# IIT-PAVIS/Acoustic-Image-Generation

Measured on AMD Instinct MI355X. Metric: train-step images/sec, higher is better.
Workload: dtype f32

## Files before the change

### acoustic-image-generation_amd/csrc/igemm.hip

```cpp
#include "wgrad_split3_kernel.hpp"
#include "igemm_split3d_kernel.hpp"
#include "igemm_split3dp_kernel.hpp"
#include "igemm_split3r_kernel.hpp"
#include "igemm_split3h_kernel.hpp"
#include "skinny_kernel.hpp"
#include <cstdlib>
#include <algorithm>
#include <type_traits>

namespace acimg {

__global__ __launch_bounds__(256) void igemm_splitk_reduce_kernel(const float* slab, int splits,
                                                                  int M, int Ngemm, int slab_ld,
                                                                  const EpiParams e) {
    const long idx = (long)blockIdx.x * 256 + threadIdx.x;
    const long total = (long)M * Ngemm;
    if (idx >= total) return;
    const int m = (int)(idx / Ngemm);
    const int n = (int)(idx - (long)m * Ngemm);
    float v = 0.f;
    for (int z = 0; z < splits; ++z) v += slab[((long)z * M + m) * slab_ld + n];
    if (n >= e.Nstore) return;
    int cn, pixoff, r, q, oh, ow;
    epi_col(e, n, cn, pixoff, r, q);
    const long rp = epi_row_pix(e, m, oh, ow);
    if (epi_lands(e, oh, ow, r, q)) epi_store(e, rp + pixoff, cn, v);
}

__global__ __launch_bounds__(256) void subpixel_weights_kernel(const float* w, int R, int S, int Ko, int Kin, int ldw, int U,
                                                               int V, float* wc, int total) {
    const int idx = blockIdx.x * 256 + threadIdx.x;
    if (idx >= total) return;
    const int ncol = 4 * Ko;
    const int row = idx / ncol, col = idx - row * ncol;
    const int kin = row % Kin, tap = row / Kin;
    const int up = tap / V, vp = tap - up * V;
    const int cls = col / Ko, ko = col - cls * Ko;
    const int a = cls >> 1, b = cls & 1;
    const int r = a + 2 * (U - 1 - up), q = b + 2 * (V - 1 - vp);
    wc[idx] = (r < R && q < S) ? w[((long)(r * S + q) * Ko + ko) * ldw + kin] : 0.f;
}

template <int BMO, int BN, int WGM = 2>
__global__ __launch_bounds__(256) void wgrad_f32_kernel(const WgradParams p) {
    constexpr int BKR = 16;
    constexpr int LDA_S = BMO + 4;
    constexpr int LDB_S = BN + 4;
    constexpr int WGN = 4 / WGM;
    constexpr int WTM = BMO / WGM, WTN = BN / WGN;
    static_assert(WTM % 16 == 0 && WTN % 16 == 0, "wave tile");
    constexpr int TM = WTM / 16, TN = WTN / 16;
    constexpr int AQ = BMO / 4;
    constexpr int ARPP = 256 / AQ;
    constexpr int NA = (BKR + ARPP - 1) / ARPP;
    constexpr int BQ = BN / 4;
    constexpr int BRPP = 256 / BQ;
    constexpr int NB = (BKR + BRPP - 1) / BRPP;

    __shared__ __attribute__((aligned(16))) float As[BKR * LDA_S];
    __shared__ __attribute__((aligned(16))) float Bs[BKR * LDB_S];

    const int tid = threadIdx.x;
    const int lane = tid & 63, wid = tid >> 6;
    const int wm = wid / WGN, wn = wid % WGN;
    const int li = lane & 15, g = lane >> 4;
    const int kk0 = blockIdx.x * BMO, n0 = blockIdx.y * BN;

    const int m_begin = blockIdx.z * p.rows_per_split;
    const int m_end = min(p.M, m_begin + p.rows_per_split);

    const int aq = tid % AQ;
    const int arow0 = tid / AQ;
    const int kk = kk0 + aq * 4;
    const bool kk_ok = kk < p.KK;
    const bool kk_ones = p.db_out != nullptr && kk == p.KK;
    int r = 0, s = 0, c = 0;
    if (kk_ok) {
        const int tap = kk / p.C;
        c = kk - tap * p.C;
        r = tap / p.S;
        s = tap - r * p.S;
    }
    const int bq = tid % BQ;
    const int brow0 = tid / BQ;
    const int nb = n0 + bq * 4;
    const bool nb_ok = nb < p.Nld;
    const int ohw = p.OH * p.OW;

    int x_img[NA], x_oh[NA], x_ow[NA];
#pragma unroll
    for (int j = 0; j < NA; ++j) {
        const int m = m_begin + arow0 + j * ARPP;
        x_img[j] = m / ohw;
        const int rem = m - x_img[j] * ohw;
        x_oh[j] = rem / p.OW;
        x_ow[j] = rem - x_oh[j] * p.OW;
    }

    float4 ra[NA], rb[NB];
    auto load_tiles = [&](int mb) {
#pragma unroll
        for (int j = 0; j < NA; ++j) {
            const int row = arow0 + j * ARPP;
            const int m = mb + row;
            float4 v = make_float4(0.f, 0.f, 0.f, 0.f);
            if (row < BKR && kk_ones && m < m_end) v.x = 1.f;
            if (row < BKR && kk_ok && m < m_end) {
                const int ih = x_oh[j] * p.stride - p.pad_t + r;
                const int iw = x_ow[j] * p.stride - p.pad_l + s;
                if ((unsigned)ih < (unsigned)p.H && (unsigned)iw < (unsigned)p.W)
                    v = *reinterpret_cast<const float4*>(
                        p.X + ((long)(x_img[j] * p.H + ih) * p.W + iw) * p.ldx + c);
            }
            ra[j] = v;
            x_ow[j] += BKR;
            while (x_ow[j] >= p.OW) {
                x_ow[j] -= p.OW;
                if (++x_oh[j] == p.OH) {
                    x_oh[j] = 0;
                    ++x_img[j];
                }
            }
        }
#pragma unroll
        for (int j = 0; j < NB; ++j) {
            const int row = brow0 + j * BRPP;
            const int m = mb + row;
            float4 v = make_float4(0.f, 0.f, 0.f, 0.f);
            if (row < BKR && nb_ok && m < m_end)
                v = *reinterpret_cast<const float4*>(p.G + (long)m * p.ldg + nb);
            rb[j] = v;
        }
    };
    auto store_tiles = [&]() {
#pragma unroll
        for (int j = 0; j < NA; ++j) {
            const int row = arow0 + j * ARPP;
            if (row < BKR) *reinterpret_cast<float4*>(&As[row * LDA_S + aq * 4]) = ra[j];
        }
#pragma unroll
        for (int j = 0; j < NB; ++j) {
            const int row = brow0 + j * BRPP;
            if (row < BKR) *reinterpret_cast<float4*>(&Bs[row * LDB_S + bq * 4]) = rb[j];
        }
    };

    f32x4 acc[TM][TN];
#pragma unroll
    for (int i = 0; i < TM; ++i)
#pragma unroll
        for (int j = 0; j < TN; ++j) acc[i][j] = f32x4{0.f, 0.f, 0.f, 0.f};

    if (m_begin < m_end) {
// ... 508 lines not shown
    if (s <= 1) return 0;
    const int ld = (Ngemm + 3) & ~3;
    const size_t rows = (size_t)s * M * ld * sizeof(float);
    const size_t tiled = (size_t)s * cdiv(M, c.bm) * cdiv(Ngemm, c.bn) * c.bm * c.bn * sizeof(float);
    return rows > tiled ? rows : tiled;
}

template <int BM, int BN, int WGM, int WGN, int NTHR>
static void launch_cfg(const IgemmParams& p, bool nt, bool cal, dim3 grid, hipStream_t st) {
    constexpr int BK = 32;
    constexpr int a_elems = BM * (BK + 4);
    constexpr int bnt = BN * (BK + 4), bnn = BK * (BN + 4);
    const int stage = a_elems + (nt ? bnt : bnn);
    const int stat_elems = WGM * 2 * BN;
    const int elems = 2 * stage > stat_elems ? 2 * stage : stat_elems;
    const size_t shm = (size_t)elems * sizeof(float);
    if (nt) {
        if (cal) hipLaunchKernelGGL((igemm_f32_kernel<BM, BN, WGM, WGN, NTHR, true, true>), grid, dim3(NTHR), shm, st, p);
        else hipLaunchKernelGGL((igemm_f32_kernel<BM, BN, WGM, WGN, NTHR, true, false>), grid, dim3(NTHR), shm, st, p);
    } else {
        if (cal) hipLaunchKernelGGL((igemm_f32_kernel<BM, BN, WGM, WGN, NTHR, false, true>), grid, dim3(NTHR), shm, st, p);
        else hipLaunchKernelGGL((igemm_f32_kernel<BM, BN, WGM, WGN, NTHR, false, false>), grid, dim3(NTHR), shm, st, p);
    }
}

static void epi_vec_flag(EpiParams& e) {
    e.vec = aligned16(e.Y) && (e.ldy & 3) == 0 && (!e.bias || aligned16(e.bias)) &&
            (!e.res || (aligned16(e.res) && (e.ldres & 3) == 0)) &&
            (!e.mask || (aligned16(e.mask) && (e.ldmask & 3) == 0)) && (!e.scatter || (e.Ko & 3) == 0);
}

static IgemmParams fwd_view(const AcimgConvDesc* d) {
    IgemmParams p{};
    p.H = d->H; p.W = d->W; p.C = d->C; p.lda = d->ldx;
    p.OH = d->OH; p.OW = d->OW; p.R = d->R; p.S = d->S; p.stride = d->stride;
    p.pad_t = d->pad_t; p.pad_l = d->pad_l;
    p.M = d->N * d->OH * d->OW;
    p.Nld = d->ldw; p.Ngemm = d->K;
    p.e.ldy = d->ldy; p.e.M = p.M; p.e.Nstore = d->K; p.e.act = d->act; p.e.stats_ld = d->ldw;
    return p;
}
static IgemmParams flipped_view(int N, int GH, int GW, int ca, int ldgy, int H, int W, int R, int S, int pad_t, int pad_l,
                                int cols) {
    IgemmParams p{};
    p.H = GH; p.W = GW; p.C = ca; p.lda = ldgy;
    p.OH = H; p.OW = W; p.R = R; p.S = S; p.stride = 1;
    p.pad_t = R - 1 - pad_t; p.pad_l = S - 1 - pad_l;
    p.M = N * H * W;
    p.Ngemm = cols;
    p.e.M = p.M; p.e.Nstore = cols; p.e.act = ACIMG_ACT_NONE;
    return p;
}
static IgemmParams flipped_view(const AcimgConvDesc* d, int ca, int ldgy) {
    return flipped_view(d->N, d->OH, d->OW, ca, ldgy, d->H, d->W, d->R, d->S, d->pad_t, d->pad_l, d->C);
}
static void split_ksteps(IgemmParams& p) {
    p.ntaps = p.R * p.S;
    p.kiters = p.ntaps * (p.C / 32);
    p.splits = 1;
}

static int launch_igemm(IgemmParams p, bool nt, void* ws, size_t ws_bytes, void* tickets, hipStream_t st) {
    if (p.M <= 0 || p.Ngemm <= 0) return fail(ACIMG_EINVAL, "igemm: empty problem");
    if ((p.C & 3) || (p.lda & 3) || (p.ldb & 3))
        return fail(ACIMG_EINVAL, "igemm: C=%d lda=%d ldb=%d must be multiples of 4", p.C, p.lda, p.ldb);
    if (!aligned16(p.A) || !aligned16(p.B)) return fail(ACIMG_EINVAL, "igemm: operands must be 16-byte aligned");
    const int nseg = p.rowrun ? p.R : p.R * p.S;
    p.L = p.rowrun ? p.S * p.C : p.C;
    p.cps = cdiv(p.L, 32);
    p.kiters = nseg * p.cps;
    p.ntaps = p.R * p.S;
    const bool cal = (p.C % 32) == 0;
    const long nimg = p.M / ((long)p.OH * p.OW);
    const long a_bytes = ((nimg * p.H * p.W - 1) * p.lda + p.C) * 4;
    const long b_bytes = nt ? (((long)(p.ntaps - 1) * p.tap_stride + (long)(p.Ngemm - 1) * p.ldb + p.C) * 4)
                            : ((long)p.R * p.S * p.C * p.ldb * 4);
    if (a_bytes >= (1L << 31) || b_bytes >= (1L << 31) || a_bytes <= 0 || b_bytes <= 0)
        return fail(ACIMG_EINVAL, "igemm: operand extent %ld / %ld bytes outside (0, 2 GiB)", a_bytes, b_bytes);
    p.a_bytes = (unsigned)a_bytes;
    p.b_bytes = (unsigned)b_bytes;
    EpiParams& e = p.e;
    epi_vec_flag(e);
    TileCfg c = pick_cfg(p.M, p.Ngemm);
    p.splits = pick_splits(p.M, p.Ngemm, c, p.kiters);
    float* stats_after = nullptr;
    if (e.stats && p.splits > 1) {
        if (e.scatter || e.res || e.mask || e.act != ACIMG_ACT_NONE)
            return fail(ACIMG_EINVAL, "igemm: statistics with split-K need a raw (conv + bias) output");
        stats_after = e.stats;
        e.stats = nullptr;
    }
    p.slab = nullptr;
    p.slab_ld = (p.Ngemm + 3) & ~3;
    p.ts_counters = nullptr;
    dim3 grid(cdiv(p.M, c.bm), cdiv(p.Ngemm, c.bn), p.splits);
    if (p.splits > 1) {
        size_t need = (size_t)p.splits * p.M * p.slab_ld * sizeof(float);
        const size_t tiles = (size_t)grid.x * grid.y;
        if (tickets && (reinterpret_cast<uintptr_t>(tickets) & 15))
            return fail(ACIMG_EINVAL, "igemm: ticket words must be 16-byte aligned");
        const bool handoff = tickets != nullptr && tiles <= ACIMG_TICKET_WORDS && g_cfg.splitk_handoff;
        if (handoff) need = (size_t)p.splits * tiles * c.bm * c.bn * sizeof(float);
        if (ws == nullptr || ws_bytes < need)
            return fail(ACIMG_EWORKSPACE, "igemm: workspace %zu < %zu", ws_bytes, need);
        p.slab = static_cast<float*>(ws);
        if (handoff) p.ts_counters = static_cast<int*>(tickets);
    }
    if (c.bm == 128 && c.bn == 128) launch_cfg<128, 128, 2, 4, 512>(p, nt, cal, grid, st);
    else if (c.bm == 128 && c.bn == 64) launch_cfg<128, 64, 2, 2, 256>(p, nt, cal, grid, st);
    else if (c.bm == 64 && c.bn == 64) launch_cfg<64, 64, 2, 2, 256>(p, nt, cal, grid, st);
    else launch_cfg<256, 16, 4, 1, 256>(p, nt, cal, grid, st);
    int rc = check_launch("igemm");
    if (rc) return rc;
    if (p.splits > 1) {
        if (p.ts_counters == nullptr) {
            const long total = (long)p.M * p.Ngemm;
            hipLaunchKernelGGL(igemm_splitk_reduce_kernel, dim3(cdiv(total, 256)), dim3(256), 0, st,
                               p.slab, p.splits, p.M, p.Ngemm, p.slab_ld, p.e);
            rc = check_launch("igemm_splitk_reduce");
        }
        if (!rc && stats_after) {
            hipLaunchKernelGGL(partial_stats_kernel, dim3(cdiv(p.M, 256)), dim3(256), 0, st, e.Y, e.ldy, p.M,
                               e.Nstore, stats_after, e.stats_ld, 256);
            rc = check_launch("partial_stats");
        }
    }
    return rc;
}

static int pick_wgrad_splits(int M, int KK, int Ngemm, int bmo, int bn) {
    const long tiles = (long)cdiv(KK, bmo) * cdiv(Ngemm, bn);
    long s = (512 + tiles - 1) / tiles;
    const int minpix = g_cfg.wgrad_minpix;
    const long maxs = (M + minpix - 1) / minpix;
    long cap = 128;
    if ((long)KK * Ngemm <= 8192) {
        s = (2048 + tiles - 1) / tiles;
        cap = 2048;
    }
    if (s > maxs) s = maxs;
    if (s > cap) s = cap;
    if (s < 1) s = 1;
    return (int)s;
}
static void wgrad_tile(int Ngemm, int& bmo, int& bn) {
    bmo = 128;
    bn = Ngemm <= 16 ? 16 : (Ngemm <= 32 ? 32 : (Ngemm <= 64 ? 64 : 128));
    if (Ngemm > 64 && cdiv(Ngemm, 64) * 64 < cdiv(Ngemm, 128) * 128) bn = 64;
}
static int wgrad_split3_bn(int Ngemm) {
    return Ngemm > 64 ? 128 : (Ngemm > 32 ? 64 : 32);
}
static bool wgrad_halo16_shape(long M, int KK, int Ngemm) { return Ngemm <= 32 && KK % 9 == 0 && KK <= 9 * 64 && M >= 65536; }
static size_t wgrad_ws_bytes(int M, int KK, int Ngemm, int ldo) {
    int bmo, bn;
    wgrad_tile(Ngemm, bmo, bn);
    int s = std::max(pick_wgrad_splits(M, KK, Ngemm, bmo, bn), pick_wgrad_splits(M, KK, Ngemm, bmo, wgrad_split3_bn(Ngemm)));
    if (wgrad_halo16_shape(M, KK, Ngemm) && s < (KK <= 9 * 16 ? 512 : 256)) s = KK <= 9 * 16 ? 512 : 256;
    return s > 1 ? (size_t)(s + 1) * ((size_t)KK + 1) * ldo * sizeof(float) : 0;
}

struct WgradHaloParams {
    const float* X; int H, W, C, ldx;
    const float* G; int OH, OW, Kp, ldg;
    int R, S, stride, pad_t, pad_l;
    int XH, XW;
    int tiles_x, tiles_y; long tiles;
    int KK;
    float* out; float* db_out; int ldo;
};
constexpr int WH_TH = 8, WH_TW = 32, WH_MAXT = 10;

template <int NT, int NKT>
__global__ __launch_bounds__(256, 3) void wgrad_halo_kernel(const WgradHaloParams p) {
    extern __shared__ __attribute__((aligned(16))) float wh_smem[];
    const int xsz = p.XH * p.XW * p.C;
    float* xs = wh_smem;
    float* gs = wh_smem + xsz + 4;
    const int tid = threadIdx.x, lane = tid & 63, wid = tid >> 6;
    const int row16 = lane & 15, quad = lane >> 4;
    int xoff[NKT], xmask[NKT];
#pragma unroll
    for (int t = 0; t < NKT; ++t) {
        const int kk = 16 * t + row16;
        if (kk < p.KK) {
            const int tap = kk / p.C, c = kk - tap * p.C;
            const int r = tap / p.S, q = tap - r * p.S;
            xoff[t] = (r * p.XW + q) * p.C + c;
            xmask[t] = -1;
        } else {
            xoff[t] = xsz + (kk == p.KK ? 0 : 1);
            xmask[t] = 0;
        }
    }
    int bcol[NT];
    float bscale[NT];
#pragma unroll
    for (int j = 0; j < NT; ++j) {
        bscale[j] = row16 + 16 * j < p.Kp ? 1.f : 0.f;
        bcol[j] = min(row16 + 16 * j, p.Kp - 1);
    }
    f32x4 acc[NKT][NT];
#pragma unroll
    for (int t = 0; t < NKT; ++t)
#pragma unroll
        for (int j = 0; j < NT; ++j) acc[t][j] = f32x4{0.f, 0.f, 0.f, 0.f};
    if (tid == 0) {
        xs[xsz] = 1.f;
        xs[xsz + 1] = 0.f;
    }
    const int c4n = p.C >> 2, k4n = p.Kp >> 2;
    const int c4sh = c4n == 1 ? 0 : (c4n == 2 ? 1 : 2);
    float4 xv[3][3], gv[2][2];
    const int rowlen = p.XW << c4sh;
    auto issue = [&](long tile) {
        const int tx = (int)(tile % p.tiles_x);
        const long t2 = tile / p.tiles_x;
        const int ty = (int)(t2 % p.tiles_y);
        const long img = t2 / p.tiles_y;
        const int oh0 = ty * WH_TH, ow0 = tx * WH_TW;
        const int ih0 = oh0 * p.stride - p.pad_t, iw0 = ow0 * p.stride - p.pad_l;
#pragma unroll
        for (int a = 0; a < 3; ++a) {
            const int iy = wid + 4 * a;
            const int ih = ih0 + iy;
            const int ihc = min(max(ih, 0), p.H - 1);
            const float* grow = p.X + ((img * p.H + ihc) * p.W) * p.ldx;
#pragma unroll
            for (int bq = 0; bq < 3; ++bq) {
                const int e = lane + 64 * bq;
                const int ix = e >> c4sh, c4 = e & (c4n - 1);
                const int iw = iw0 + ix;
                const bool ok = iy < p.XH && e < rowlen && (unsigned)ih < (unsigned)p.H && (unsigned)iw < (unsigned)p.W;
                const float4 v = *reinterpret_cast<const float4*>(grow + (long)min(max(iw, 0), p.W - 1) * p.ldx + 4 * c4);
                xv[a][bq] = ok ? v : make_float4(0.f, 0.f, 0.f, 0.f);
            }
        }
#pragma unroll
        for (int half = 0; half < 2; ++half) {
            const int py = 2 * wid + half, px = lane & 31;
            const int oh = oh0 + py, ow = ow0 + px;
            const bool ok = oh < p.OH && ow < p.OW;
            const float* gsrc = p.G + ((img * p.OH + min(oh, p.OH - 1)) * p.OW + min(ow, p.OW - 1)) * p.ldg;
#pragma unroll
            for (int j = 0; j < 2; ++j) {
                const int k4 = (lane >> 5) + 2 * j;
                const float4 v = *reinterpret_cast<const float4*>(gsrc + 4 * min(k4, k4n - 1));
                gv[half][j] = ok && k4 < k4n ? v : make_float4(0.f, 0.f, 0.f, 0.f);
            }
        }
    };
    auto commit = [&]() {
#pragma unroll
        for (int a = 0; a < 3; ++a) {
            const int iy = wid + 4 * a;
#pragma unroll
            for (int bq = 0; bq < 3; ++bq) {
                const int e = lane + 64 * bq;
                if (iy < p.XH && e < rowlen)
                    *reinterpret_cast<float4*>(xs + iy * p.XW * p.C + (e >> c4sh) * p.C + 4 * (e & (c4n - 1))) = xv[a][bq];
            }
        }
#pragma unroll
        for (int half = 0; half < 2; ++half)
#pragma unroll
            for (int j = 0; j < 2; ++j) {
                const int k4 = (lane >> 5) + 2 * j;
                if (k4 < k4n)
                    *reinterpret_cast<float4*>(gs + ((2 * wid + half) * WH_TW + (lane & 31)) * p.Kp + 4 * k4) = gv[half][j];
            }
    };
    issue(blockIdx.x);
    for (long tile = blockIdx.x; tile < p.tiles; tile += gridDim.x) {
        __syncthreads();
        commit();
        __syncthreads();
        if (tile + gridDim.x < p.tiles) issue(tile + gridDim.x);
        {
            int xb = ((2 * wid) * p.XW + quad) * p.C;
            const float* gp = gs + ((2 * wid) * WH_TW + quad) * p.Kp;
            float a[2][NKT], b[2][NT];
#pragma unroll
            for (int t = 0; t < NKT; ++t) a[0][t] = xs[xoff[t] + (xb & xmask[t])];
#pragma unroll
            for (int j = 0; j < NT; ++j) b[0][j] = gp[bcol[j]] * bscale[j];
#pragma unroll 1
            for (int g2 = 0; g2 < 8; ++g2) {
#pragma unroll
                for (int cur = 0; cur < 2; ++cur) {
                    const int nxt = cur ^ 1;
                    const int gq = 2 * g2 + cur;
                    if (gq < 15) {
                        gp += 4 * p.Kp;
                        xb += 4 * p.C + (gq == 7 ? (p.XW - WH_TW) * p.C : 0);
#pragma unroll
                        for (int t = 0; t < NKT; ++t) a[nxt][t] = xs[xoff[t] + (xb & xmask[t])];
#pragma unroll
                        for (int j = 0; j < NT; ++j) b[nxt][j] = gp[bcol[j]] * bscale[j];
                    }
#pragma unroll
                    for (int t = 0; t < NKT; ++t)
#pragma unroll
                        for (int j = 0; j < NT; ++j)
                            acc[t][j] = __builtin_amdgcn_mfma_f32_16x16x4f32(a[cur][t], b[cur][j], acc[t][j], 0, 0, 0);
                }
            }
// ... 81 lines not shown
        gb[h] = (jh * TW + col) * 64 + (((2 * nt + (pp >> 1)) ^ swg(col)) << 4) + 8 * (pp & 1);
#pragma unroll
        for (int s_ = 0; s_ < 3; ++s_) {
            const int cx = col + s_;
            xb[s_][h] = (jh * XW + cx) * PITCH + (((2 * ct + (pp >> 1)) ^ swx(cx)) << 4) + 8 * (pp & 1);
        }
    }

    float4 rx[NXL], rg[NGL];
    unsigned okm = 0;
    const bool aff_ch = p.a_scale != nullptr && (tid % (C / 4)) * 4 < p.creal;
    const float4 asc = aff_ch ? *reinterpret_cast<const float4*>(p.a_scale + (tid % (C / 4)) * 4) : make_float4(1.f, 1.f, 1.f, 1.f);
    const float4 ash = aff_ch ? *reinterpret_cast<const float4*>(p.a_shift + (tid % (C / 4)) * 4) : make_float4(0.f, 0.f, 0.f, 0.f);
    auto load_tile = [&](long tile) {
        okm = 0;
        const int tx = (int)(tile % p.tiles_x);
        const long t2 = tile / p.tiles_x;
        const int ty = (int)(t2 % p.tiles_y);
        const long img = t2 / p.tiles_y;
        const float* xi = p.X + img * p.H * p.W * p.ldx;
        const float* gi = p.G + img * p.H * p.W * p.ldg;
#pragma unroll
        for (int k = 0; k < NXL; ++k) {
            const int i = tid + 512 * k;
            const int c4 = i % (C / 4), pix = i / (C / 4);
            const int row = pix / XWV, col = pix - row * XWV;
            const int iy = ty * TH + row - 1, ix = tx * TW + col - 1;
            float4 v = make_float4(0.f, 0.f, 0.f, 0.f);
            if (row < XH && c4 * 4 < p.creal && (unsigned)iy < (unsigned)p.H && (unsigned)ix < (unsigned)p.W) {
                v = *reinterpret_cast<const float4*>(xi + ((long)iy * p.W + ix) * p.ldx + c4 * 4);
                okm |= 1u << k;
            }
            rx[k] = v;
        }
#pragma unroll
        for (int k = 0; k < NGL; ++k) {
            const int i = tid + 512 * k;
            const int c4 = i & 7, pix = i >> 3;
            const int row = pix / TW, col = pix - row * TW;
            const int oy = ty * TH + row, ox = tx * TW + col;
            float4 v = make_float4(0.f, 0.f, 0.f, 0.f);
            if (oy < p.H && ox < p.W && c4 * 4 < p.nreal) v = *reinterpret_cast<const float4*>(gi + ((long)oy * p.W + ox) * p.ldg + c4 * 4);
            rg[k] = v;
        }
    };
    auto store_tile = [&]() {
#pragma unroll
        for (int k = 0; k < NXL; ++k) {
            const int i = tid + 512 * k;
            const int c4 = i % (C / 4), pix = i / (C / 4);
            const int row = pix / XWV, col = pix - row * XWV;
            if (row < XH) {
                const int off = (row * XW + col) * PITCH + (((c4 >> 1) ^ swx(col)) << 4) + 8 * (c4 & 1);
                uint2 hi, lo;
                split4<SplitBF16>(p.a_scale && ((okm >> k) & 1u) ? affine_relu4(rx[k], asc, ash, p.a_relu != 0) : rx[k], hi, lo);
                *reinterpret_cast<uint2*>(lds + off) = hi;
                if (TERMS == 3) *reinterpret_cast<uint2*>(lds + XPL + off) = lo;
            }
        }
#pragma unroll
        for (int k = 0; k < NGL; ++k) {
            const int i = tid + 512 * k;
            const int c4 = i & 7, pix = i >> 3;
            const int col = pix & (TW - 1);
            const int off = pix * 64 + (((c4 >> 1) ^ swg(col)) << 4) + 8 * (c4 & 1);
            uint2 hi, lo;
            split4<SplitBF16>(rg[k], hi, lo);
            *reinterpret_cast<uint2*>(gl + off) = hi;
            if (TERMS == 3) *reinterpret_cast<uint2*>(gl + GPL + off) = lo;
        }
    };
    typedef short s16x4_ __attribute__((ext_vector_type(4)));
    typedef short s16x8_ __attribute__((ext_vector_type(8)));
    auto frag = [&](const char* base, int a0, int a1) -> b16x8 {
        const s16x4_ v0 = __builtin_amdgcn_ds_read_tr16_b64_v4i16((__attribute__((address_space(3))) s16x4_*)(base + a0));
        const s16x4_ v1 = __builtin_amdgcn_ds_read_tr16_b64_v4i16((__attribute__((address_space(3))) s16x4_*)(base + a1));
        const s16x8_ v = {v0[0], v0[1], v0[2], v0[3], v1[0], v1[1], v1[2], v1[3]};
        return __builtin_bit_cast(b16x8, v);
    };

    f32x4 acc[9], accb = {0.f, 0.f, 0.f, 0.f};
#pragma unroll
    for (int t = 0; t < 9; ++t) acc[t] = f32x4{0.f, 0.f, 0.f, 0.f};
    const __bf16 one = (__bf16)1.f;
    const b16x8 ones = {one, one, one, one, one, one, one, one};

    long tile = blockIdx.x;
    if (tile < p.tiles) load_tile(tile);
    for (; tile < p.tiles; tile += gridDim.x) {
        __syncthreads();
        store_tile();
        __syncthreads();
        if (tile + gridDim.x < p.tiles) load_tile(tile + gridDim.x);
#pragma unroll
        for (int jj = 0; jj < TH / NJ; ++jj) {
            const int j = jj * NJ;
            const b16x8 gh = frag(gl + j * TW * 64, gb[0], gb[1]);
            b16x8 glo;
            if (TERMS == 3) glo = frag(gl + GPL + j * TW * 64, gb[0], gb[1]);
#pragma unroll
            for (int r = 0; r < 3; ++r)
#pragma unroll
                for (int s_ = 0; s_ < 3; ++s_) {
                    const char* xrow = lds + (j + r) * XW * PITCH;
                    const b16x8 xh = frag(xrow, xb[s_][0], xb[s_][1]);
                    if (TERMS == 3) {
                        const b16x8 xl = frag(xrow + XPL, xb[s_][0], xb[s_][1]);
                        acc[r * 3 + s_] = SplitBF16::mfma(glo, xh, acc[r * 3 + s_]);
                        acc[r * 3 + s_] = SplitBF16::mfma(gh, xl, acc[r * 3 + s_]);
                    }
                    acc[r * 3 + s_] = SplitBF16::mfma(gh, xh, acc[r * 3 + s_]);
                }
            if (ct == 0) {
                if (TERMS == 3) accb = SplitBF16::mfma(glo, ones, accb);
                accb = SplitBF16::mfma(gh, ones, accb);
            }
        }
    }
    if (NJ > 1) {
        f32x4* red = reinterpret_cast<f32x4*>(lds);
        const int w0 = wid % (NCT * NNT);
        for (int r = 1; r < NJ; ++r) {
            __syncthreads();
            if (jh == r) {
#pragma unroll
                for (int t = 0; t < 9; ++t) red[(w0 * 10 + t) * 64 + lane] = acc[t];
                red[(w0 * 10 + 9) * 64 + lane] = accb;
            }
            __syncthreads();
            if (jh == 0) {
#pragma unroll
                for (int t = 0; t < 9; ++t) acc[t] += red[(w0 * 10 + t) * 64 + lane];
                accb += red[(w0 * 10 + 9) * 64 + lane];
            }
        }
        if (jh != 0) return;
    }
    float* out = p.out + (long)blockIdx.x * (9 * p.creal) * p.ldo;
    const bool nok = nt * 16 + 4 * g < p.nreal;
    if (nok && ct * 16 + li < p.creal) {
#pragma unroll
        for (int t = 0; t < 9; ++t)
            *reinterpret_cast<f32x4*>(out + (long)(t * p.creal + ct * 16 + li) * p.ldo + nt * 16 + 4 * g) = acc[t];
    }
    if (p.db_out && ct == 0 && li == 0 && nok)
        *reinterpret_cast<f32x4*>(p.db_out + (long)blockIdx.x * p.ldo + nt * 16 + 4 * g) = accb;
}

static bool wgrad_halo16_ok(const WgradParams& p, bool split3) {
    const bool few = p.C < 32;
    return wgrad_halo16_shape(p.M, p.KK, p.Ngemm) && (split3 || few) && p.R == 3 && p.S == 3 && p.stride == 1 && p.pad_t == 1 &&
           p.pad_l == 1 && (p.C == 64 || (p.C <= 32 && p.C % 4 == 0)) && p.Ngemm % 4 == 0 && p.Nld == p.Ngemm && p.OH == p.H &&
           p.OW == p.W && p.ldo >= p.Ngemm && g_cfg.wgrad_halo;
}

static int launch_wgrad(WgradParams p, float* dw, float* db, void* ws, size_t ws_bytes, hipStream_t st,
                        bool split3 = false, int terms = 3) {
    if ((p.C & 3) || (p.ldx & 3) || (p.ldg & 3) || (p.ldo & 3))
        return fail(ACIMG_EINVAL, "wgrad: C=%d ldx=%d ldg=%d ldo=%d must be multiples of 4", p.C, p.ldx, p.ldg, p.ldo);
    if (!aligned16(p.X) || !aligned16(p.G) || !aligned16(dw))
        return fail(ACIMG_EINVAL, "wgrad: operands must be 16-byte aligned");
    if (p.a_scale && !wgrad_halo16_ok(p, split3))
        return fail(ACIMG_EINVAL, "wgrad: an input affine is only taken by the halo form (3x3 / stride 1 / SAME, <= 32 columns, >= 65536 pixels)");
    if (p.a_scale && (!p.a_shift || !aligned16(p.a_scale) || !aligned16(p.a_shift)))
        return fail(ACIMG_EINVAL, "wgrad: the input affine needs scale and shift, 16-byte aligned");
    int bmo, bn;
    wgrad_tile(p.Ngemm, bmo, bn);
    if (wgrad_halo16_ok(p, split3)) {
        WgradHalo16Params q{};
        q.X = p.X; q.H = p.H; q.W = p.W; q.ldx = p.ldx; q.G = p.G; q.ldg = p.ldg; q.ldo = p.ldo;
        q.creal = p.C; q.nreal = p.Ngemm;
        q.a_scale = p.a_scale; q.a_shift = p.a_shift; q.a_relu = p.a_relu;
        if (p.C < 32) terms = 3;
        const int cpad = p.C == 64 ? 64 : (p.C > 16 ? 32 : 16);
        const int nnt = (cpad == 16 && p.Ngemm <= 16) ? 1 : 2;
        const int th = (terms == 1 || cpad == 16) ? 8 : 4;
        q.tiles_x = cdiv(p.W, 32); q.tiles_y = cdiv(p.H, th);
        q.tiles = (long)(p.M / (p.H * p.W)) * q.tiles_x * q.tiles_y;
        int nb = p.C <= 16 ? 512 : 256;
        if (nb > q.tiles) nb = (int)q.tiles;
        const size_t need = (size_t)nb * ((size_t)p.KK + 1) * p.ldo * sizeof(float);
        if (ws != nullptr && ws_bytes >= need) {
            q.out = static_cast<float*>(ws);
            float* db_slab = q.out + (size_t)nb * p.KK * p.ldo;
            q.db_out = db ? db_slab : nullptr;
            const int xh = th + 2, planes = terms == 3 ? 2 : 1;
            int lds = planes * (xh * 36 * cpad * 2 + th * 32 * 64);
            if (lds < 4 * 10 * 64 * 16) lds = 4 * 10 * 64 * 16;
#define ACIMG_WH16(Cv, Tv)                                                                                              \
    do {                                                                                                                \
        static bool attr_set = false;                                                                                   \
        if (!attr_set) {                                                                                                \
            (void)hipFuncSetAttribute(reinterpret_cast<const void*>(wgrad_halo16_kernel<Cv, Tv>),                       \
                                      hipFuncAttributeMaxDynamicSharedMemorySize, 2 * (10 * 36 * 64 * 2 + 8 * 32 * 64)); \
            attr_set = true;                                                                                            \
        }                                                                                                               \
        hipLaunchKernelGGL((wgrad_halo16_kernel<Cv, Tv>), dim3(nb), dim3(512), lds, st, q);                             \
    } while (0)
            if (cpad == 64 && terms == 1) ACIMG_WH16(64, 1);
            else if (cpad == 64) ACIMG_WH16(64, 3);
            else if (cpad == 32 && terms == 1) ACIMG_WH16(32, 1);
            else if (cpad == 32) ACIMG_WH16(32, 3);
            else if (nnt == 2) ACIMG_WH16(16, 3);
            else {
                static bool attr16 = false;
                if (!attr16) {
                    (void)hipFuncSetAttribute(reinterpret_cast<const void*>(wgrad_halo16_kernel<16, 3, 1>),
                                              hipFuncAttributeMaxDynamicSharedMemorySize, 65536);
                    attr16 = true;
                }
                hipLaunchKernelGGL((wgrad_halo16_kernel<16, 3, 1>), dim3(nb), dim3(512), lds, st, q);
            }
#undef ACIMG_WH16
            int rc = check_launch("wgrad_halo16");
            if (rc) return rc;
            launch_slab_reduce_wide(q.out, nb, (long)p.KK, p.Ngemm, p.ldo, dw, db ? db_slab : nullptr, db, st);
            return check_launch("wgrad_reduce");
        }
    }
    if (p.a_scale) return fail(ACIMG_EWORKSPACE, "wgrad: workspace too small for the halo form, which the input affine needs");
    if (wgrad_halo_ok(p)) {
        WgradHaloParams q{};
        q.X = p.X; q.H = p.H; q.W = p.W; q.C = p.C; q.ldx = p.ldx;
        q.G = p.G; q.OH = p.OH; q.OW = p.OW; q.Kp = p.Nld; q.ldg = p.ldg;
        q.R = p.R; q.S = p.S; q.stride = p.stride; q.pad_t = p.pad_t; q.pad_l = p.pad_l;
        q.XH = (WH_TH - 1) * p.stride + p.R; q.XW = (WH_TW - 1) * p.stride + p.S;
        q.tiles_x = cdiv(p.OW, WH_TW); q.tiles_y = cdiv(p.OH, WH_TH);
        q.tiles = (long)(p.M / (p.OH * p.OW)) * q.tiles_x * q.tiles_y;
        q.KK = p.KK; q.ldo = p.ldo;
        int nb = pick_wgrad_splits(p.M, p.KK, p.Ngemm, bmo, bn);
        if (nb > 768) nb = 768;
        if (nb > q.tiles) nb = (int)q.tiles;
        if (nb < 2) nb = 2;
        const size_t need = (size_t)nb * ((size_t)p.KK + 1) * p.ldo * sizeof(float);
        if (ws == nullptr || ws_bytes < need) return fail(ACIMG_EWORKSPACE, "wgrad: workspace %zu < %zu", ws_bytes, need);
        q.out = static_cast<float*>(ws);
        float* db_slab = q.out + (size_t)nb * p.KK * p.ldo;
        q.db_out = db ? db_slab : nullptr;
        const size_t lds = wgrad_halo_lds(p.R, p.S, p.C, p.Nld, p.stride);
        const int nkt = (p.KK + 1 + 15) / 16;
#define ACIMG_WH(NTv, NKTv) hipLaunchKernelGGL((wgrad_halo_kernel<NTv, NKTv>), dim3(nb), dim3(256), lds, st, q)
        if (nkt <= 1) ACIMG_WH(1, 1);
        else if (nkt <= 2) ACIMG_WH(1, 2);
        else if (nkt <= 3) ACIMG_WH(1, 3);
        else if (nkt <= 5) ACIMG_WH(1, 5);
        else ACIMG_WH(1, 10);
#undef ACIMG_WH
        int rc = check_launch("wgrad_halo");
        if (rc) return rc;
        launch_slab_reduce_wide(q.out, nb, (long)p.KK, p.Ngemm, p.ldo, dw, db ? db_slab : nullptr, db, st);
        return check_launch("wgrad_reduce");
    }
    if (split3) bn = wgrad_split3_bn(p.Ngemm);
    p.splits = pick_wgrad_splits(p.M, p.KK, p.Ngemm, bmo, bn);
    int rps = cdiv(p.M, p.splits);
    rps = ((rps + 31) / 32) * 32;
    p.rows_per_split = rps;
    p.splits = cdiv(p.M, rps);
    float* db_slab = nullptr;
    if (p.splits > 1) {
        const size_t need = (size_t)p.splits * ((size_t)p.KK + 1) * p.ldo * sizeof(float);
        if (ws == nullptr || ws_bytes < need)
            return fail(ACIMG_EWORKSPACE, "wgrad: workspace %zu < %zu", ws_bytes, need);
        p.out = static_cast<float*>(ws);
        db_slab = p.out + (size_t)p.splits * p.KK * p.ldo;
        p.db_out = db ? db_slab : nullptr;
    } else {
        p.out = dw;
        p.db_out = db;
    }
    const int rows = p.KK + (db ? 1 : 0);
    dim3 grid(cdiv(rows, bmo), cdiv(p.Ngemm, bn), p.splits);
    if (split3 && terms == 1 && bn == 128) hipLaunchKernelGGL((wgrad_split3_kernel<128, 1, 512>), grid, dim3(512), 65536, st, p);
    else if (split3 && terms == 1 && bn == 64) hipLaunchKernelGGL((wgrad_split3_kernel<64, 1, 512>), grid, dim3(512), 65536, st, p);
    else if (split3 && terms == 1) hipLaunchKernelGGL((wgrad_split3_kernel<32, 1>), grid, dim3(256), 65536, st, p);
    else if (split3 && bn == 128) hipLaunchKernelGGL((wgrad_split3_kernel<128, 3, 512>), grid, dim3(512), 65536, st, p);
    else if (split3 && bn == 64) hipLaunchKernelGGL((wgrad_split3_kernel<64, 3, 512>), grid, dim3(512), 65536, st, p);
    else if (split3) hipLaunchKernelGGL((wgrad_split3_kernel<32>), grid, dim3(256), 65536, st, p);
    else if (bn == 128) hipLaunchKernelGGL((wgrad_f32_kernel<128, 128>), grid, dim3(256), 0, st, p);
    else if (bn == 64) hipLaunchKernelGGL((wgrad_f32_kernel<128, 64>), grid, dim3(256), 0, st, p);
    else if (bn == 32) hipLaunchKernelGGL((wgrad_f32_kernel<128, 32>), grid, dim3(256), 0, st, p);
    else hipLaunchKernelGGL((wgrad_f32_kernel<128, 16, 4>), grid, dim3(256), 0, st, p);
    int rc = check_launch("wgrad");
    if (rc) return rc;
    if (p.splits > 1) {
        const long total = (long)p.KK * p.Ngemm;
        if (p.splits > 32) {
            launch_slab_reduce_wide(p.out, p.splits, (long)p.KK, p.Ngemm, p.ldo, dw, db ? db_slab : nullptr, db, st);
        } else {
            const int nb1 = (int)cdiv(total, 256), nb2 = db ? cdiv(p.Ngemm, 256) : 0;
            hipLaunchKernelGGL(slab_reduce_kernel, dim3(nb1 + nb2), dim3(256), 0, st, p.out, p.splits,
                               (long)p.KK, p.Ngemm, p.ldo, dw, nb1, db_slab, db);
        }
        rc = check_launch("wgrad_reduce");
    }
    return rc;
}

static int colsum_parts(long rows) {
    int parts = (int)((rows + 255) / 256);
    if (parts > 256) parts = 256;
    if (parts < 1) parts = 1;
    return parts;
}
static int launch_colsum(const float* G, long rows, int ncols, int ld, float* out, void* ws,
                         size_t ws_bytes, hipStream_t st) {
    const int parts = colsum_parts(rows);
    const long rpb = (rows + parts - 1) / parts;
    const size_t need = (size_t)parts * ncols * sizeof(float);
    if (ws == nullptr || ws_bytes < need) return fail(ACIMG_EWORKSPACE, "colsum: workspace %zu < %zu", ws_bytes, need);
    float* partial = static_cast<float*>(ws);
    if (ncols <= 64 && (ncols & 3) == 0 && (ld & 3) == 0 && aligned16(G))
        hipLaunchKernelGGL(colsum_narrow_kernel, dim3(parts), dim3(256), 0, st, G, rows, ncols, ld, rpb, partial);
    else
        hipLaunchKernelGGL(colsum_partial_kernel, dim3(cdiv(ncols, 64), parts), dim3(256), 0, st, G, rows,
                           ncols, ld, rpb, partial);
    hipLaunchKernelGGL(colsum_final_kernel, dim3(cdiv(ncols, 64)), dim3(256), 0, st, partial, parts, ncols, out);
    return check_launch("colsum");
}
static size_t colsum_ws_bytes(int ncols) { return (size_t)256 * ncols * sizeof(float); }

static int check_desc(const AcimgConvDesc* d, const char* who, bool row_run = false) {
    if (!d) return fail(ACIMG_EINVAL, "%s: null descriptor", who);
    if (d->N <= 0 || d->H <= 0 || d->W <= 0 || d->C <= 0 || d->K <= 0 || d->OH <= 0 || d->OW <= 0 ||
        d->R <= 0 || d->S <= 0 || d->stride <= 0)
        return fail(ACIMG_EINVAL, "%s: non-positive dimension", who);
    const bool run_view = row_run && d->S == 1 && d->pad_l == 0 && d->ldx > 0 && d->C % d->ldx == 0 &&
                          (d->OW - 1) * d->stride + d->C / d->ldx <= d->W;
    if ((d->C & 3) || (d->ldx & 3) || (d->ldw & 3) || (d->ldx < d->C && !run_view))
        return fail(ACIMG_EINVAL, "%s: C=%d ldx=%d ldw=%d must be multiples of 4 (ldx>=C)", who, d->C, d->ldx, d->ldw);
    if ((long)d->N * d->H * d->W * d->ldx >= (1L << 31) || (long)d->N * d->OH * d->OW * (long)d->ldy >= (1L << 31))
        return fail(ACIMG_EINVAL, "%s: tensor exceeds 2^31 elements", who);
    return ACIMG_OK;
}
static inline int up4(int v) { return (v + 3) & ~3; }

static bool direct_shape(int C, int K) { return C <= 16 && K <= 32; }
static bool direct_ok(int C, int K, int ldy, int ldres, const float* y, const float* bias, const float* res,
                      bool affine, const float* mask) {
    return !affine && !mask && direct_shape(C, K) && ldy >= ((K + 3) & ~3) && (C & 3) == 0 && (ldy & 3) == 0 &&
           (!res || ((ldres & 3) == 0 && aligned16(res))) && aligned16(y) && (!bias || aligned16(bias));
}
static size_t direct_ws_bytes(int R, int S, int C, int K) { return ((size_t)R * S * C * K * sizeof(float) + 255) & ~(size_t)255; }
static int launch_direct(const DirectParams& q, void* ws, size_t ws_bytes, hipStream_t st) {
    if (!aligned16(q.x) || (q.ldx & 3)) return fail(ACIMG_EINVAL, "direct conv: input must be 16-byte aligned");
    const int total = q.R * q.S * q.C * ((q.K + 7) & ~7);
    if (!ws || ws_bytes < (size_t)total * sizeof(float)) return fail(ACIMG_EWORKSPACE, "direct conv: workspace too small");
    float* wprep = static_cast<float*>(ws);
    hipLaunchKernelGGL(direct_prepare_kernel, dim3(cdiv(total, 256)), dim3(256), 0, st, q, wprep, total);
    const long units = (long)cdiv(q.M, 256) * cdiv(q.K, 8);
    const dim3 grid((unsigned)(8 * ((units + 7) / 8)));
#define ACIMG_DIRECT(RR, SS, CC) \
    hipLaunchKernelGGL((direct_conv_kernel<RR, SS, CC>), grid, dim3(256), 0, st, q, wprep)
    if (q.R == 3 && q.S == 3 && q.C == 4) ACIMG_DIRECT(3, 3, 4);
    else if (q.R == 3 && q.S == 3 && q.C == 8) ACIMG_DIRECT(3, 3, 8);
    else if (q.R == 3 && q.S == 3 && q.C == 16) ACIMG_DIRECT(3, 3, 16);
    else if (q.R == 1 && q.S == 1 && q.C == 8) ACIMG_DIRECT(1, 1, 8);
    else if (q.R == 2 && q.S == 2 && q.C == 8) ACIMG_DIRECT(2, 2, 8);
    else ACIMG_DIRECT(0, 0, 0);
#undef ACIMG_DIRECT
    return check_launch("direct_conv");
}

struct FewParams {
    const float* X; int H, W, ldx;
    int Hin, Win, SH, SW, dil, pad_t, pad_l;
    const char* Wimg; unsigned w_lo_off;
    float* Y; int ldy, nout;
    const float* bias; const float* res; int ldres;
    float* stats; int stats_ld;
    int tiles_x, tiles_y; long tiles, per;
    const float* a_scale; const float* a_shift; int a_relu;
    const float* w; int ldw, wrows, cin, mode;
};
constexpr int FEW16_WGS = 512;
constexpr int few16_ktot(int cin) { return ((9 + 32 / cin - 1) / (32 / cin)) * 32; }

template <typename TR>
__global__ __launch_bounds__(256) void few16_prepare_kernel(const FewParams p, int CIN, int NOUTP, typename TR::T* img) {
    typedef typename TR::T T;
    const int KTOT = few16_ktot(CIN);
    const int i = blockIdx.x * 256 + threadIdx.x;
    if (i >= NOUTP * KTOT) return;
    const int row = i / KTOT, k = i - row * KTOT;
    const int slot = k / CIN, c = k - slot * CIN;
    float v = 0.f;
    if (slot < 9 && row < p.nout && c < p.cin)
        v = p.mode == 0 ? p.w[((long)slot * p.wrows + c) * p.ldw + row] : p.w[((long)(8 - slot) * p.wrows + row) * p.ldw + c];
    v *= TR::WSCALE;
    const T h = (T)v;
    img[i] = h;
    img[(size_t)NOUTP * KTOT + i] = (T)(v - (float)h);
}

template <typename TR, int CIN, int NOUTP, int MODE, int CLOAD = CIN>
__global__ __launch_bounds__(512, (NOUTP == 32 && MODE == 0) ? 2 : 4) void conv_few16_kernel(const FewParams p) {
    typedef typename TR::V8 V8;
    constexpr int TH = 16, TW = 32, XH = TH + 2, XWV = TW + 2, XW = 36;
    constexpr int PB = CIN * 2;
    constexpr int XPL = XH * XW * PB;
    constexpr int TPK = 32 / CIN;
    constexpr int NKB = (9 + TPK - 1) / TPK;
    constexpr int KTOT = NKB * 32;
    constexpr int NT = NOUTP / 16;
    constexpr int NXL = (XH * XWV * (CLOAD / 4) + 511) / 512;
    static_assert((CIN == 8 || CIN == 16) && (CLOAD == CIN || (CIN == 8 && CLOAD == 4)), "few-channel instance");
// ... 1740 lines not shown
```

Baseline: 5086.

## Add tap-reuse weight-gradient kernel for wide 3x3 stride-1 convolutions

```diff
diff --git a/acoustic-image-generation_amd/csrc/igemm.hip b/acoustic-image-generation_amd/csrc/igemm.hip
--- a/acoustic-image-generation_amd/csrc/igemm.hip
+++ b/acoustic-image-generation_amd/csrc/igemm.hip
@@ -1,4 +1,5 @@
 #include "wgrad_split3_kernel.hpp"
+#include "wgrad_tap_kernel.hpp"
 #include "igemm_split3d_kernel.hpp"
 #include "igemm_split3dp_kernel.hpp"
 #include "igemm_split3r_kernel.hpp"
@@ -813,6 +814,7 @@
     return Ngemm > 64 ? 128 : (Ngemm > 32 ? 64 : 32);
 }
 static bool wgrad_halo16_shape(long M, int KK, int Ngemm) { return Ngemm <= 32 && KK % 9 == 0 && KK <= 9 * 64 && M >= 65536; }
+static bool wgrad_tap_shape(int KK, int Ngemm) { return KK % 9 == 0 && KK >= 9 * 64 && Ngemm > 32; }
 static size_t wgrad_ws_bytes(int M, int KK, int Ngemm, int ldo) {
     int bmo, bn;
     wgrad_tile(Ngemm, bmo, bn);
@@ -1200,6 +1202,12 @@
     return wgrad_halo16_shape(p.M, p.KK, p.Ngemm) && (split3 || few) && p.R == 3 && p.S == 3 && p.stride == 1 && p.pad_t == 1 &&
            p.pad_l == 1 && (p.C == 64 || (p.C <= 32 && p.C % 4 == 0)) && p.Ngemm % 4 == 0 && p.Nld == p.Ngemm && p.OH == p.H &&
            p.OW == p.W && p.ldo >= p.Ngemm && g_cfg.wgrad_halo;
+}
+
+static bool wgrad_tap_ok(const WgradParams& p) {
+    return wgrad_tap_shape(p.KK, p.Ngemm) && p.R == 3 && p.S == 3 && p.stride == 1 && p.pad_t == 1 && p.pad_l == 1 &&
+           p.OH == p.H && p.OW == p.W && p.W % 16 == 0 && p.W >= 32 && p.W <= WT_MAXW && p.KK == 9 * p.C && p.Nld == p.Ngemm &&
+           p.Ngemm % 4 == 0 && p.ldo >= p.Ngemm && p.M % (p.H * p.W) == 0 && !p.a_scale && g_cfg.wgrad_halo;
 }
 
 static int launch_wgrad(WgradParams p, float* dw, float* db, void* ws, size_t ws_bytes, hipStream_t st,
@@ -1300,6 +1308,49 @@
         return check_launch("wgrad_reduce");
     }
     if (split3) bn = wgrad_split3_bn(p.Ngemm);
+    if (split3 && terms == 3 && wgrad_tap_ok(p)) {
+        WgradTapParams q{};
+        q.X = p.X; q.H = p.H; q.W = p.W; q.C = p.C; q.ldx = p.ldx; q.G = p.G; q.ldg = p.ldg;
+        q.Ngemm = p.Ngemm; q.Nld = p.Nld; q.KK = p.KK; q.ldo = p.ldo;
+        q.tiles_y = cdiv(p.H, WT_TH);
+        q.tiles = (long)(p.M / (p.H * p.W)) * q.tiles_y;
+        int ns = pick_wgrad_splits(p.M, p.KK, p.Ngemm, bmo, bn);
+        if (ns > q.tiles) ns = (int)q.tiles;
+        float* db_slab = nullptr;
+        if (ns > 1) {
+            const size_t need = (size_t)ns * ((size_t)p.KK + 1) * p.ldo * sizeof(float);
+            if (ws == nullptr || ws_bytes < need) return fail(ACIMG_EWORKSPACE, "wgrad: workspace %zu < %zu", ws_bytes, need);
+            q.out = static_cast<float*>(ws);
+            db_slab = q.out + (size_t)ns * p.KK * p.ldo;
+            q.db_out = db ? db_slab : nullptr;
+        } else {
+            q.out = dw;
+            q.db_out = db;
+        }
+        const size_t lds = wgrad_tap_lds(p.W);
+        static bool attr_set = false;
+        if (!attr_set) {
+            (void)hipFuncSetAttribute(reinterpret_cast<const void*>(wgrad_tap_kernel<128>), hipFuncAttributeMaxDynamicSharedMemorySize,
+                                      (int)wgrad_tap_lds(WT_MAXW));
+            (void)hipFuncSetAttribute(reinterpret_cast<const void*>(wgrad_tap_kernel<64>), hipFuncAttributeMaxDynamicSharedMemorySize,
+                                      (int)wgrad_tap_lds(WT_MAXW));
+            attr_set = true;
+        }
+        const dim3 grid(cdiv(p.C, WT_CB), cdiv(p.Ngemm, bn), ns);
+        if (bn == 128) hipLaunchKernelGGL((wgrad_tap_kernel<128>), grid, dim3(512), lds, st, q);
+        else hipLaunchKernelGGL((wgrad_tap_kernel<64>), grid, dim3(512), lds, st, q);
+        int rc = check_launch("wgrad_tap");
+        if (rc || ns == 1) return rc;
+        if (ns > 32) {
+            launch_slab_reduce_wide(q.out, ns, (long)p.KK, p.Ngemm, p.ldo, dw, db ? db_slab : nullptr, db, st);
+        } else {
+            const long total = (long)p.KK * p.Ngemm;
+            const int nb1 = (int)cdiv(total, 256), nb2 = db ? cdiv(p.Ngemm, 256) : 0;
+            hipLaunchKernelGGL(slab_reduce_kernel, dim3(nb1 + nb2), dim3(256), 0, st, q.out, ns, (long)p.KK, p.Ngemm, p.ldo, dw, nb1,
+                               db_slab, db);
+        }
+        return check_launch("wgrad_reduce");
+    }
     p.splits = pick_wgrad_splits(p.M, p.KK, p.Ngemm, bmo, bn);
     int rps = cdiv(p.M, p.splits);
     rps = ((rps + 31) / 32) * 32;
diff --git a/acoustic-image-generation_amd/csrc/wgrad_tap_kernel.hpp b/acoustic-image-generation_amd/csrc/wgrad_tap_kernel.hpp
--- /dev/null
+++ b/acoustic-image-generation_amd/csrc/wgrad_tap_kernel.hpp
@@ -0,0 +1,198 @@
+#pragma once
+#include "wgrad_split3_kernel.hpp"
+
+namespace acimg {
+
+struct WgradTapParams {
+    const float* X; int H, W, C, ldx;
+    const float* G; int ldg;
+    int Ngemm, Nld;
+    int tiles_y; long tiles;
+    int KK;
+    float* out; float* db_out; int ldo;
+};
+
+constexpr int WT_TH = 2, WT_CB = 32, WT_MAXW = 48;
+static inline size_t wgrad_tap_lds(int W) { return (size_t)512 * (W + 2) + (size_t)1024 * W; }
+
+template <int NB>
+__global__ __launch_bounds__(512) void wgrad_tap_kernel(const WgradTapParams p) {
+    constexpr int TH = WT_TH, XH = TH + 2, CB = WT_CB;
+    constexpr int TNW = NB / 64;
+    constexpr int GQ = NB / 4;
+    constexpr int NXL = (XH * (WT_MAXW + 2) * (CB / 4) + 511) / 512;
+    constexpr int NGL = TH * WT_MAXW * GQ / 512;
+    static_assert(NB == 128 || NB == 64, "column block");
+    extern __shared__ __attribute__((aligned(16))) float wt_smem[];
+    char* const lds = reinterpret_cast<char*>(wt_smem);
+    const int XW = p.W + 2, npix = TH * p.W;
+    const int XPL = XH * XW * 64;
+    const int GPL = npix * 256;
+    char* const xh_pl = lds;
+    char* const xl_pl = lds + XPL;
+    char* const gh_pl = lds + 2 * XPL;
+    char* const gl_pl = gh_pl + GPL;
+
+    const int tid = threadIdx.x, lane = tid & 63, wid = tid >> 6;
+    const int li = lane & 15, g = lane >> 4, q = li >> 2, pp = li & 3;
+    const int ct = wid & 1, ng = wid >> 1;
+    const int c0 = blockIdx.x * CB, n0 = blockIdx.y * NB;
+    const long t_begin = (long)blockIdx.z * p.tiles / gridDim.z, t_end = (long)(blockIdx.z + 1) * p.tiles / gridDim.z;
+
+    int x_row[NXL], x_goff[NXL], x_lds[NXL];
+#pragma unroll
+    for (int k = 0; k < NXL; ++k) {
+        const int i = tid + 512 * k;
+        const int c4 = i & 7, pix = i >> 3;
+        const int row = pix / XW, col = pix - row * XW;
+        const bool ok = row < XH && col >= 1 && col <= p.W && c0 + c4 * 4 < p.C;
+        x_row[k] = row < XH ? (ok ? row - 1 : 1 << 20) : -(1 << 20);
+        x_goff[k] = ((row - 1) * p.W + col - 1) * p.ldx + c0 + c4 * 4;
+        x_lds[k] = (row * XW + col) * 64 + (((c4 >> 1) ^ (2 * ((col >> 3) & 1))) << 4) + 8 * (c4 & 1);
+    }
+    const int gq = tid % GQ, gpix0 = tid / GQ;
+    const bool gn_ok = n0 + gq * 4 < p.Nld;
+
+    float4 rx[NXL], rg[NGL];
+    auto load_tile = [&](long tile) {
+        const long img = tile / p.tiles_y;
+        const int y0 = (int)(tile - img * p.tiles_y) * TH;
+        const float* xi = p.X + (img * p.H + y0) * (long)p.W * p.ldx;
+        const float* gi = p.G + (img * p.H + y0) * (long)p.W * p.ldg + n0 + gq * 4;
+        const int left = (p.H - y0) * p.W;
+#pragma unroll
+        for (int k = 0; k < NXL; ++k) {
+            float4 v = make_float4(0.f, 0.f, 0.f, 0.f);
+            if ((unsigned)(y0 + x_row[k]) < (unsigned)p.H) v = *reinterpret_cast<const float4*>(xi + x_goff[k]);
+            rx[k] = v;
+        }
+#pragma unroll
+        for (int k = 0; k < NGL; ++k) {
+            const int pix = gpix0 + k * (512 / GQ);
+            float4 v = make_float4(0.f, 0.f, 0.f, 0.f);
+            if (gn_ok && pix < npix && pix < left) v = *reinterpret_cast<const float4*>(gi + (long)pix * p.ldg);
+            rg[k] = v;
+        }
+    };
+    auto store_tile = [&]() {
+#pragma unroll
+        for (int k = 0; k < NXL; ++k) {
+            if (x_row[k] > -(1 << 20)) {
+                uint2 hi, lo;
+                split4<SplitBF16>(rx[k], hi, lo);
+                *reinterpret_cast<uint2*>(xh_pl + x_lds[k]) = hi;
+                *reinterpret_cast<uint2*>(xl_pl + x_lds[k]) = lo;
+            }
+        }
+#pragma unroll
+        for (int k = 0; k < NGL; ++k) {
+            const int pix = gpix0 + k * (512 / GQ);
+            if (pix < npix) {
+                const int f = (pix & 3) | (((pix >> 3) & 1) << 2);
+                const int off = pix * 256 + (((gq >> 2) ^ f) << 5) + ((gq & 3) << 3);
+                uint2 hi, lo;
+                split4<SplitBF16>(rg[k], hi, lo);
+                *reinterpret_cast<uint2*>(gh_pl + off) = hi;
+                *reinterpret_cast<uint2*>(gl_pl + off) = lo;
+            }
+        }
+    };
+    typedef short s16x8 __attribute__((ext_vector_type(8)));
+    auto xfrag = [&](const char* base, int a0, int a1) -> b16x8 {
+        const s16x4 v0 = __builtin_amdgcn_ds_read_tr16_b64_v4i16((__attribute__((address_space(3))) s16x4*)(base + a0));
+        const s16x4 v1 = __builtin_amdgcn_ds_read_tr16_b64_v4i16((__attribute__((address_space(3))) s16x4*)(base + a1));
+        const s16x8 v = {v0[0], v0[1], v0[2], v0[3], v1[0], v1[1], v1[2], v1[3]};
+        return __builtin_bit_cast(b16x8, v);
+    };
+
+    f32x4 acc[9][TNW], accb[TNW];
+#pragma unroll
+    for (int i = 0; i < TNW; ++i) {
+        accb[i] = f32x4{0.f, 0.f, 0.f, 0.f};
+#pragma unroll
+        for (int t = 0; t < 9; ++t) acc[t][i] = f32x4{0.f, 0.f, 0.f, 0.f};
+    }
+    const __bf16 one = (__bf16)1.f;
+    const b16x8 ones = {one, one, one, one, one, one, one, one};
+    const bool bias_wave = p.db_out != nullptr && blockIdx.x == 0 && ct == 0;
+    const int nks = npix >> 5;
+    const int xcb = 2 * ct + (pp >> 1), xsub = 8 * (pp & 1);
+    const int rowb = XW * 64;
+
+    long tile = t_begin;
+    if (tile < t_end) load_tile(tile);
+    for (; tile < t_end; ++tile) {
+        __syncthreads();
+        store_tile();
+        __syncthreads();
+        if (tile + 1 < t_end) load_tile(tile + 1);
+        int orow = 0, ocol = 8 * g + q;
+        for (int ks = 0; ks < nks; ++ks) {
+            while (ocol >= p.W) { ocol -= p.W; ++orow; }
+            int xa[3][2];
+#pragma unroll
+            for (int s_ = 0; s_ < 3; ++s_)
+#pragma unroll
+                for (int h = 0; h < 2; ++h) {
+                    const int cx = ocol + 4 * h + s_;
+                    xa[s_][h] = (orow * XW + cx) * 64 + ((xcb ^ (2 * ((cx >> 3) & 1))) << 4) + xsub;
+                }
+            b16x8 gh[TNW], gl[TNW];
+#pragma unroll
+            for (int i = 0; i < TNW; ++i) {
+                const int colbyte = ((ng * TNW + i) * 16) * 2;
+                gh[i] = tr_frag(gh_pl + ks * 8192, 8 * g, colbyte, lane);
+                gl[i] = tr_frag(gl_pl + ks * 8192, 8 * g, colbyte, lane);
+            }
+#pragma unroll
+            for (int r = 0; r < 3; ++r)
+#pragma unroll
+                for (int s_ = 0; s_ < 3; ++s_) {
+                    const b16x8 xh = xfrag(xh_pl + r * rowb, xa[s_][0], xa[s_][1]);
+                    const b16x8 xl = xfrag(xl_pl + r * rowb, xa[s_][0], xa[s_][1]);
+#pragma unroll
+                    for (int i = 0; i < TNW; ++i) {
+                        acc[r * 3 + s_][i] = SplitBF16::mfma(gl[i], xh, acc[r * 3 + s_][i]);
+                        acc[r * 3 + s_][i] = SplitBF16::mfma(gh[i], xl, acc[r * 3 + s_][i]);
+                        acc[r * 3 + s_][i] = SplitBF16::mfma(gh[i], xh, acc[r * 3 + s_][i]);
+                    }
+                }
+            if (bias_wave) {
+#pragma unroll
+                for (int i = 0; i < TNW; ++i) {
+                    accb[i] = SplitBF16::mfma(gl[i], ones, accb[i]);
+                    accb[i] = SplitBF16::mfma(gh[i], ones, accb[i]);
+                }
+            }
+            ocol += 32;
+        }
+    }
+
+    float* out = p.out + (long)blockIdx.z * p.KK * p.ldo;
+    const int c = c0 + ct * 16 + li;
+#pragma unroll
+    for (int i = 0; i < TNW; ++i) {
+        const int n = n0 + (ng * TNW + i) * 16 + 4 * g;
+        if (n >= p.Ngemm) continue;
+        const bool whole = n + 3 < p.Ngemm;
+        if (c < p.C) {
+#pragma unroll
+            for (int t = 0; t < 9; ++t) {
+                float* dst = out + (long)(t * p.C + c) * p.ldo + n;
+                if (whole) *reinterpret_cast<f32x4*>(dst) = acc[t][i];
+                else
+                    for (int k = 0; k < 4; ++k)
+                        if (n + k < p.Ngemm) dst[k] = acc[t][i][k];
+            }
+        }
+        if (bias_wave && li == 0) {
+            float* dst = p.db_out + (long)blockIdx.z * p.ldo + n;
+            if (whole) *reinterpret_cast<f32x4*>(dst) = accb[i];
+            else
+                for (int k = 0; k < 4; ++k)
+                    if (n + k < p.Ngemm) dst[k] = accb[i][k];
+        }
+    }
+}
+
+}
```

New measurement: 5184, median of 6. +1.9%, better.
